# segasai/rvspecfit

Measured on AMD Instinct MI355X. Metric: spectra/sec (CCF+chi2 grid) DESI 3-arm, higher is better.
Workload: dtype f64

## Files before the change

rvspecfit_amd/csrc/ccf.hip:

```cpp
#include "common.h"

#define PP_NT 512
#define PP_LOG2NT 9
#define PP_NW (PP_NT / 64)


#define SEL_NB PP_NT
struct SelShared {
  unsigned long long kmin, kmax, result, next, cand[64];
  int hist[SEL_NB];
  int wtot[PP_NW];
  int cnt, nnan, nc, bucket, kk, nle;
};
__device__ __forceinline__ unsigned long long sel_key(double x) {
  const unsigned long long b = (unsigned long long)__double_as_longlong(x);
  return (b >> 63) ? ~b : (b | 0x8000000000000000ull);
}
__device__ __forceinline__ double sel_value(unsigned long long k) {
  const unsigned long long b = (k >> 63) ? (k & 0x7fffffffffffffffull) : ~k;
  return __longlong_as_double((long long)b);
}
__device__ __forceinline__ unsigned long long shfl_xor_u64(unsigned long long v,
                                                           int o) {
  const int lo = __shfl_xor((int)(v & 0xffffffffu), o, 64);
  const int hi = __shfl_xor((int)(v >> 32), o, 64);
  return ((unsigned long long)(unsigned)hi << 32) | (unsigned)lo;
}

__device__ double block_median(const double *v, int n, bool skipnan,
                               SelShared &Q) {
  const int tid = threadIdx.x, lane = tid & 63, wv = tid >> 6;
  {
    int cnt = 0, nn = 0;
    unsigned long long mn = ~0ull, mx = 0ull;
    for (int k = tid; k < n; k += PP_NT) {
      const double x = v[k];
      if (x != x) {
        nn++;
        continue;
      }
      const unsigned long long key = sel_key(x);
      cnt++;
      mn = key < mn ? key : mn;
      mx = key > mx ? key : mx;
    }
    cnt = wave_sum_i(cnt);
    nn = wave_sum_i(nn);
#pragma unroll
    for (int o = 32; o > 0; o >>= 1) {
      const unsigned long long a = shfl_xor_u64(mn, o), b = shfl_xor_u64(mx, o);
      mn = a < mn ? a : mn;
      mx = b > mx ? b : mx;
    }
    if (tid == 0) {
      Q.cnt = 0;
      Q.nnan = 0;
      Q.kmin = ~0ull;
      Q.kmax = 0ull;
    }
    __syncthreads();
    if (lane == 0) {
      atomicAdd(&Q.cnt, cnt);
      atomicAdd(&Q.nnan, nn);
      atomicMin(&Q.kmin, mn);
      atomicMax(&Q.kmax, mx);
    }
    __syncthreads();
  }
  const int nval = Q.cnt;
  if (nval == 0 || (!skipnan && Q.nnan > 0)) {
    __syncthreads();
    return __builtin_nan("");
  }
  const int k_lo = (nval - 1) >> 1, k_hi = nval >> 1;
  unsigned long long lo = Q.kmin, range = Q.kmax - Q.kmin;
  int kk = k_lo, ncand = nval;
  __syncthreads();
  unsigned long long found = 0;
  bool done = false;
  if (range == 0) {
    found = lo;
    done = true;
  }
  while (!done) {
    const int bits = 64 - __clzll((long long)range);
    const int shift = bits > PP_LOG2NT ? bits - PP_LOG2NT : 0;
    if (ncand <= 64) {
      if (tid == 0) Q.nc = 0;
      __syncthreads();
      for (int k = tid; k < n; k += PP_NT) {
        const double x = v[k];
        if (x != x) continue;
        const unsigned long long key = sel_key(x);
        if (key >= lo && key - lo <= range) Q.cand[atomicAdd(&Q.nc, 1)] = key;
      }
      __syncthreads();
      if (wv == 0) {
        const int nc = Q.nc;
        const unsigned long long my = lane < nc ? Q.cand[lane] : ~0ull;
        int lt = 0, eq = 0;
        for (int j = 0; j < nc; j++) {
          const unsigned long long c = Q.cand[j];
          lt += c < my;
          eq += c == my;
        }
        if (lane < nc && lt <= kk && kk < lt + eq) Q.result = my;
      }
      __syncthreads();
      found = Q.result;
      break;
    }
    Q.hist[tid] = 0;
    __syncthreads();
    for (int k = tid; k < n; k += PP_NT) {
      const double x = v[k];
      if (x != x) continue;
      const unsigned long long key = sel_key(x);
      if (key >= lo && key - lo <= range)
        atomicAdd(&Q.hist[(int)((key - lo) >> shift)], 1);
    }
    __syncthreads();
    const int h = Q.hist[tid];
    int inc = h;
#pragma unroll
    for (int o = 1; o < 64; o <<= 1) {
      const int t = __shfl_up(inc, o, 64);
      if (lane >= o) inc += t;
    }
    if (lane == 63) Q.wtot[wv] = inc;
    __syncthreads();
    int off = 0;
    for (int w = 0; w < wv; w++) off += Q.wtot[w];
    inc += off;
    if (inc - h <= kk && kk < inc) {
      Q.bucket = tid;
      Q.kk = kk - (inc - h);
      Q.nc = h;
    }
    __syncthreads();
    const int bsel = Q.bucket;
    kk = Q.kk;
    ncand = Q.nc;
    lo += (unsigned long long)bsel << shift;
    if (shift == 0) {
      found = lo;
      break;
    }
    range = (1ull << shift) - 1;
    __syncthreads();
  }
  double med = sel_value(found);
  if (k_hi != k_lo) {
    int nle = 0;
    unsigned long long nx = ~0ull;
    for (int k = tid; k < n; k += PP_NT) {
      const double x = v[k];
      if (x != x) continue;
      const unsigned long long key = sel_key(x);
      if (key <= found)
        nle++;
      else
        nx = key < nx ? key : nx;
    }
    nle = wave_sum_i(nle);
#pragma unroll
    for (int o = 32; o > 0; o >>= 1) {
      const unsigned long long a = shfl_xor_u64(nx, o);
      nx = a < nx ? a : nx;
    }
    __syncthreads();
    if (tid == 0) {
      Q.nle = 0;
      Q.next = ~0ull;
    }
    __syncthreads();
    if (lane == 0) {
      atomicAdd(&Q.nle, nle);
      atomicMin(&Q.next, nx);
    }
    __syncthreads();
    const double hi = (Q.nle >= k_hi + 1) ? med : sel_value(Q.next);
    med = (med + hi) * 0.5;
  }
  __syncthreads();
  return med;
}

__device__ __forceinline__ double wave_median256(const double (&x)[4], int cnt) {
  const int lane = threadIdx.x & 63;
  unsigned long long key[4];
  bool anynan = false;
#pragma unroll
  for (int h = 0; h < 4; h++) {
    const bool valid = lane + 64 * h < cnt;
    anynan |= valid && (x[h] != x[h]);
    key[h] = valid ? sel_key(x[h]) : ~0ull;
  }
  if (cnt <= 0 || __ballot(anynan) != 0ull) return __builtin_nan("");
  const int k_lo = (cnt - 1) >> 1, k_hi = cnt >> 1;
  unsigned long long p = 0;
  for (int bit = 63; bit >= 0; bit--) {
    const unsigned long long trial = p | (1ull << bit);
    int c = 0;
#pragma unroll
    for (int h = 0; h < 4; h++) c += __popcll(__ballot(key[h] < trial));
    if (c <= k_lo) p = trial;
  }
  double med = sel_value(p);
  if (k_hi != k_lo) {
    int cle = 0;
    unsigned long long nx = ~0ull;
#pragma unroll
    for (int h = 0; h < 4; h++) {
      const bool valid = lane + 64 * h < cnt;
      cle += __popcll(__ballot(valid && key[h] <= p));
      if (valid && key[h] > p && key[h] < nx) nx = key[h];
    }
#pragma unroll
    for (int o = 32; o > 0; o >>= 1) {
      const unsigned long long a = shfl_xor_u64(nx, o);
      nx = a < nx ? a : nx;
    }
    const double hi = (cle >= k_hi + 1) ? med : sel_value(nx);
    med = (med + hi) * 0.5;
  }
  return med;
}

__device__ __forceinline__ double median11_net(const double *w) {
  double a[11];
#pragma unroll
  for (int i = 0; i < 11; i++) a[i] = w[i];
#define CE(i, j)                         \
  {                                      \
    const double lo_ = fmin(a[i], a[j]); \
    a[j] = fmax(a[i], a[j]);             \
    a[i] = lo_;                          \
  }
  CE(0, 9) CE(1, 6) CE(2, 4) CE(3, 7) CE(5, 8)
  CE(0, 1) CE(3, 5) CE(4, 10) CE(6, 9) CE(7, 8)
  CE(1, 3) CE(2, 5) CE(4, 7) CE(8, 10)
  CE(0, 4) CE(1, 2) CE(3, 7) CE(5, 9) CE(6, 8)
  CE(2, 6) CE(4, 5) CE(7, 8)
  CE(2, 4) CE(3, 6) CE(5, 7)
  CE(3, 4) CE(5, 6)
  CE(4, 5)
#undef CE
  return a[5];
}

__device__ __forceinline__ double median11(double *a) {
#pragma unroll
  for (int i = 1; i < 11; i++) {
    const double x = a[i];
    int j = i - 1;
    while (j >= 0 && a[j] > x) {
      a[j + 1] = a[j];
      j--;
    }
    a[j + 1] = x;
  }
  return a[5];
}

#ifdef RVS_PP_TIMING
__device__ unsigned long long pp_dbg[16];
#define PP_T(i)                                                  \
  do {                                                           \
    __syncthreads();                                             \
    if (threadIdx.x == 0) {                                      \
      const unsigned long long t_ = wall_clock64();              \
      atomicAdd(&pp_dbg[i], t_ - t_prev);                        \
      t_prev = t_;                                               \
    }                                                            \
  } while (0)
extern "C" int rvs_dbg_read_pp(unsigned long long *out) {
  return hipMemcpyFromSymbol(out, HIP_SYMBOL(pp_dbg), sizeof(pp_dbg)) ==
                 hipSuccess
             ? 0
             : -1;
}
#define PP_TPARAM , unsigned long long &t_prev
#define PP_TPASS , t_prev
#else
#define PP_T(i)
#define PP_TPARAM
#define PP_TPASS
#endif

#define CCF_MAXNODE 24
#ifndef RVS_LM_MAXIT
#define RVS_LM_MAXIT 60
#endif

#define CCF_MODEL_MAXNODE 48
template <int MN>
struct LMSharedT {
  double p[MN];
  double c[MN], cn[MN], dl[MN];
  double bvec[MN];
  double Bd[MN * 3];
  double Lb[MN * 3];
  double isum[MN * 9];
  double red[PP_NW];
  double lamd, medv, mederr, medspec;
  int flag, ngood, firstgood, lastgood, nval, stop, ok;
};
typedef LMSharedT<CCF_MAXNODE> LMShared;
struct ErrArray {
  const double *ce;
  __device__ __forceinline__ double operator()(int k, double) const { return ce[k]; }
};


struct LMPix {
  double e0, e1, e2;
  int l;
};
#ifndef LM_PIX
#define LM_PIX 1
#endif

template <class LM, class ERR>
__device__ __forceinline__ double lm_eval(
    LM &S, const double *cc, const double *__restrict__ Eb,
    const int32_t *__restrict__ El, int npix, const double *cs, const ERR ce,
    double *wm, bool store, const LMPix (&px)[LM_PIX]) {
  __syncthreads();
  double c = 0;
#pragma unroll
  for (int i = 0; i < LM_PIX; i++) {
    const int k = threadIdx.x + i * PP_NT;
    if (k < npix) {
      const int l = px[i].l;
      double s = px[i].e0 * cc[l];
      s = fma(px[i].e1, cc[l + 1], s);
      s = fma(px[i].e2, cc[l + 2], s);
      const bool clipped = (s < -100.0) || (s > 100.0);
      s = fmin(fmax(s, -100.0), 100.0);
      const double mod = exp(s);
      const double sk = cs[k], e = ce(k, sk);
      const double f = (mod - sk) / e;
      const double z = f * f;
      const double r = sqrt(1 + z);
      c += 2 * (r - 1);
      if (store) wm[k] = clipped ? 0.0 : mod;
    }
  }
  for (int k = threadIdx.x + LM_PIX * PP_NT; k < npix; k += PP_NT) {
    const int l = El[k];
    double s = Eb[3 * k] * cc[l];
    s = fma(Eb[3 * k + 1], cc[l + 1], s);
    s = fma(Eb[3 * k + 2], cc[l + 2], s);
    const bool clipped = (s < -100.0) || (s > 100.0);
    s = fmin(fmax(s, -100.0), 100.0);
    const double mod = exp(s);
    const double sk = cs[k], e = ce(k, sk);
    const double f = (mod - sk) / e;
    const double z = f * f;
    const double r = sqrt(1 + z);
    c += 2 * (r - 1);
    if (store) wm[k] = clipped ? 0.0 : mod;
  }
  return 0.5 * block_sum<PP_NW>(c, S.red);
}

template <class LM, class ERR>
__device__ void lm_normal(LM &S, const double *__restrict__ Eb,
                          const int32_t *__restrict__ istart, int m,
                          const double *wm, const double *cs, const ERR ce) {
  const int nint = m - 2;
  const int lane = threadIdx.x & 63, wave = threadIdx.x >> 6;
  __syncthreads();
  for (int t = wave; t < nint; t += PP_NW) {
    double a[9];
#pragma unroll
    for (int q = 0; q < 9; q++) a[q] = 0;
    const int k1 = istart[t + 1];
    for (int k0 = istart[t] + lane; k0 < k1; k0 += 4 * 64) {
      double e[4][3];
#pragma unroll
      for (int c = 0; c < 4; c++) {
        const int k = min(k0 + 64 * c, k1 - 1);
        e[c][0] = Eb[3 * k];
        e[c][1] = Eb[3 * k + 1];
        e[c][2] = Eb[3 * k + 2];
      }
#pragma unroll
      for (int c = 0; c < 4; c++) {
        const int k = k0 + 64 * c;
        if (k < k1) {
          const double e0 = e[c][0], e1 = e[c][1], e2 = e[c][2];
          const double mod = wm[k], sk = cs[k], e = ce(k, sk);
          const double f = (mod - sk) / e;
          const double z = f * f;
          const double r = sqrt(1 + z);
          const double d = mod / e;
          const double h = d * d / (r * r * r), gg = d * f / r;
          a[0] = fma(h * e0, e0, a[0]);
          a[1] = fma(h * e0, e1, a[1]);
          a[2] = fma(h * e0, e2, a[2]);
          a[3] = fma(h * e1, e1, a[3]);
          a[4] = fma(h * e1, e2, a[4]);
          a[5] = fma(h * e2, e2, a[5]);
          a[6] = fma(gg, e0, a[6]);
          a[7] = fma(gg, e1, a[7]);
          a[8] = fma(gg, e2, a[8]);
        }
      }
    }
#pragma unroll
    for (int q = 0; q < 9; q++) {
      const double v = wave_sum_to63(a[q]);
      if (lane == 63) S.isum[t * 9 + q] = v;
    }
  }
  __syncthreads();
  for (int e = threadIdx.x; e < 4 * m; e += PP_NT) {
    const int a = e >> 2, d = e & 3;
    if (d == 3) {
      double s = 0;
      for (int t = max(0, a - 2); t <= min(a, nint - 1); t++)
        s += S.isum[t * 9 + 6 + (a - t)];
      S.bvec[a] = s;
    } else {
      const int lo = a - d;
      double s = 0;
      if (lo >= 0) {
        for (int t = max(0, a - 2); t <= min(lo, nint - 1); t++) {
          const int u = lo - t, v = a - t;
          const int idx = (u == 0) ? v : (u == 1 ? 2 + v : 5);
          s += S.isum[t * 9 + idx];
        }
      }
      S.Bd[a * 3 + d] = s;
    }
  }
  __syncthreads();
}

__device__ inline double lane_get(double v, int src) {
  return __hiloint2double(__builtin_amdgcn_readlane(__double2hiint(v), src),
                          __builtin_amdgcn_readlane(__double2loint(v), src));
}
__device__ inline double lane_put(double dst, double v, int lane) {
  return ((int)(threadIdx.x & 63) == lane) ? v : dst;
}

template <class LM>
__device__ void lm_band_solve(LM &S, int m) {
  const int lane = threadIdx.x & 63;
  const int r = min(lane, m - 1);
  const double ld = 1.0 + S.lamd;
  const double ra0 = S.Bd[r * 3] * ld, ra1 = S.Bd[r * 3 + 1],
               ra2 = S.Bd[r * 3 + 2], rb = S.bvec[r];
  double d1 = 0, d2 = 0, l1p = 0;
  double r1 = 0, r2 = 0;
  double z1 = 0, z2 = 0;
  double lb1 = 0, lb2 = 0, w = 0;
  bool ok = true;
  for (int i = 0; i < m; i++) {
    const double a0 = lane_get(ra0, i), a1 = lane_get(ra1, i),
                 a2 = lane_get(ra2, i), bi = lane_get(rb, i);
    const double l2 = (i >= 2) ? a2 * r2 : 0.0;
    const double l1 = (i >= 1) ? (a1 - l2 * l1p * d2) * r1 : 0.0;
    const double d = a0 - l1 * l1 * d1 - l2 * l2 * d2;
    if (!(d > 0)) ok = false;
    const double z = -bi - l1 * z1 - l2 * z2;
    const double rd = 1.0 / d;
    lb1 = lane_put(lb1, l1, i);
    lb2 = lane_put(lb2, l2, i);
    w = lane_put(w, z * rd, i);
    d2 = d1;
    d1 = d;
    r2 = r1;
    r1 = rd;
    l1p = l1;
    z2 = z1;
    z1 = z;
  }
  double x1 = 0, x2 = 0;
  double xs = 0;
  for (int i = m - 1; i >= 0; i--) {
    const double l1n = (i + 1 < m) ? lane_get(lb1, i + 1) : 0.0;
    const double l2n = (i + 2 < m) ? lane_get(lb2, i + 2) : 0.0;
    const double x = lane_get(w, i) - l1n * x1 - l2n * x2;
    xs = lane_put(xs, x, i);
    x2 = x1;
    x1 = x;
  }
  if (lane < m) {
    const double dl = ok ? xs : 0.0;
    S.dl[lane] = dl;
    S.cn[lane] = S.c[lane] + dl;
  }
  if (lane == 0) S.ok = ok ? 1 : 0;
}

template <class LM>
__device__ __forceinline__ void lm_binned_start(LM &S, SelShared &Q, const double *cs,
                                                const int32_t *__restrict__ bin_start,
                                                int m, bool f32) {
  const int tid = threadIdx.x;
  bool small = true;
  for (int jb = 0; jb < m; jb++)
    if (bin_start[jb + 1] - bin_start[jb] > 256) small = false;
  if (small) {
    const int lane = tid & 63, wv = tid >> 6;
    for (int jb = wv; jb < m; jb += PP_NW) {
      const int b0 = bin_start[jb], cnt = bin_start[jb + 1] - b0;
      double x[4];
#pragma unroll
      for (int h = 0; h < 4; h++) {
        const int q = lane + 64 * h;
        x[h] = (q < cnt) ? cs[b0 + q] : 0.0;
      }
      double stat = wave_median256(x, cnt);
      if (f32) stat = (double)(float)stat;
      if (lane == 0) {
        double p0 = log(fmax(stat, 1e-3 * S.medspec));
        if (!(stat == stat)) p0 = stat;
        if (!(fabs(p0) <= 1.79e308)) p0 = log(S.medspec);
        S.p[jb] = p0;
      }
    }
  } else {
    for (int jb = 0; jb < m; jb++) {
      const int b0 = bin_start[jb], cnt = bin_start[jb + 1] - b0;
      double stat = block_median(cs + b0, cnt, false, Q);
      if (f32) stat = (double)(float)stat;
      if (tid == 0) {
        double p0 = log(fmax(stat, 1e-3 * S.medspec));
        if (!(stat == stat)) p0 = stat;
        if (!(fabs(p0) <= 1.79e308)) p0 = log(S.medspec);
        S.p[jb] = p0;
      }
    }
  }
  __syncthreads();
}

template <class LM, class ERR>
__device__ __forceinline__ void lm_fit(LM &S, const double *__restrict__ Eb,
                                       const int32_t *__restrict__ El,
                                       const double *__restrict__ Cinv,
                                       const int32_t *__restrict__ istart, int m,
                                       int npix, const double *cs, const ERR ce,
                                       double *wm PP_TPARAM) {
  const int tid = threadIdx.x;
  if (tid < m) {
    double s = 0;
    for (int jj = 0; jj < m; jj++) s = fma(Cinv[tid * m + jj], S.p[jj], s);
    S.c[tid] = s;
  }
  if (tid == 0) {
#ifndef RVS_LM_LAMBDA0
#define RVS_LM_LAMBDA0 1e-3
#endif
    S.lamd = RVS_LM_LAMBDA0;
    S.stop = 0;
  }
  LMPix px[LM_PIX];
#pragma unroll
  for (int i = 0; i < LM_PIX; i++) {
    const int k = min(tid + i * PP_NT, npix - 1);
    px[i].e0 = Eb[3 * k];
    px[i].e1 = Eb[3 * k + 1];
    px[i].e2 = Eb[3 * k + 2];
    px[i].l = El[k];
  }
  double cost = lm_eval(S, S.c, Eb, El, npix, cs, ce, wm, true, px);
  PP_T(7);
  for (int it = 0; it < RVS_LM_MAXIT; it++) {
    lm_normal(S, Eb, istart, m, wm, cs, ce);
    PP_T(8);
    if (it == 0) {
      if (tid < 64) {
        double g = 0;
        if (tid < m)
          for (int i = 0; i < m; i++) g = fma(Cinv[i * m + tid], S.bvec[i], g);
        g = fabs(g);
        if (!(g == g)) g = 1.0;
        for (int o = 32; o > 0; o >>= 1) g = fmax(g, __shfl_xor(g, o));
        if (tid == 0 && g < 1e-8) S.stop = 1;
      }
      __syncthreads();
      if (S.stop) break;
    }
    bool accepted = false;
    for (int tries = 0; tries < 40; tries++) {
      if (tid < 64) lm_band_solve(S, m);
      PP_T(9);
      const double cn =
          lm_eval(S, S.cn, Eb, El, npix, cs, ce, wm, true, px);
      PP_T(10);
      if (cn <= cost) {
        accepted = true;
        double mx = 0;
        for (int i = 0; i < m; i++) mx = fmax(mx, fabs(S.dl[i]));
        const double rel = (cost - cn) / fmax(cost, 1e-300);
        __syncthreads();
        if (tid == 0) {
          for (int i = 0; i < m; i++) S.c[i] = S.cn[i];
          S.lamd = fmax(S.lamd / 8, 1e-12);
          if (mx < 1e-9 || rel < 1e-12) S.stop = 1;
        }
        cost = cn;
        break;
      }
      __syncthreads();
      if (tid == 0) {
        S.lamd *= 4;
        if (S.lamd > 1e12) S.stop = 1;
      }
      __syncthreads();
      if (S.stop) break;
    }
    __syncthreads();
    if (S.stop) break;
    if (!accepted)
      cost = lm_eval(S, S.c, Eb, El, npix, cs, ce, wm, true, px);
    PP_T(11);
  }
  __syncthreads();
}

__global__ void __launch_bounds__(PP_NT)
    __attribute__((amdgpu_waves_per_eu(4, 4)))
    ccf_preprocess_kernel(const double *__restrict__ lam,
                          const double *__restrict__ spec,
                          const double *__restrict__ espec,
                          const uint8_t *__restrict__ badmask, int npix,
                          int continuum, const double *__restrict__ Eb,
                          const int32_t *__restrict__ El,
                          const double *__restrict__ Cinv,
                          const int32_t *__restrict__ istart, int nnode,
                          const int32_t *__restrict__ bin_start,
                          const int32_t *__restrict__ xind,
                          const double *__restrict__ rw, int nfft, double maxerr,
                          double *__restrict__ proc_spec,
                          double *__restrict__ proc_ivar, double *__restrict__ sse,
                          double *__restrict__ cont_out,
                          double *__restrict__ pfit, int32_t *__restrict__ status,
                          const int32_t *__restrict__ gid,
                          const int32_t *__restrict__ npix_g,
                          const int32_t *__restrict__ nnode_g) {
  extern __shared__ double sm[];
  const int npix_s = npix, nnode_s = nnode;
  if (gid) {
    const int g = gid[blockIdx.x];
    npix = npix_g[g];
    nnode = nnode_g[g];
    lam += (int64_t)g * npix_s;
    xind += (int64_t)g * nfft;
    rw += (int64_t)g * nfft;
    if (continuum) {
      Eb += (int64_t)g * 3 * npix_s;
      El += (int64_t)g * npix_s;
      Cinv += (int64_t)g * 2 * nnode_s * nnode_s;
      istart += (int64_t)g * nnode_s;
      bin_start += (int64_t)g * (nnode_s + 1);
    }
  }
  double *cs = sm;
  double *ce = cs + npix;
  double *wm = ce + npix;
  uint8_t *msk = reinterpret_cast<uint8_t *>(wm + npix);
  __shared__ LMShared S;
  __shared__ SelShared Q;
  const int b = blockIdx.x, tid = threadIdx.x;
  const double *sp0 = spec + (int64_t)b * npix_s;
  const double *es0 = espec + (int64_t)b * npix_s;
#ifdef RVS_PP_TIMING
  unsigned long long t_prev = wall_clock64();
#endif

  for (int k = tid; k < npix; k += PP_NT) {
    cs[k] = sp0[k];
    ce[k] = es0[k];
    msk[k] = badmask ? (badmask[(int64_t)b * npix_s + k] != 0) : 0;
  }
  if (tid == 0) {
    S.flag = 0;
    S.nval = 0;
  }
  __syncthreads();

  {
    const double me = block_median(ce, npix, true, Q);
    if (tid == 0) S.mederr = me;
    __syncthreads();
  }
  const double mederr = S.mederr;

  if (continuum) {
    for (int k = tid; k < npix; k += PP_NT) {
      double w[11];
#pragma unroll
      for (int q = 0; q < 11; q++) {
        const int idx = k + q - 5;
        w[q] = (idx >= 0 && idx < npix) ? cs[idx] : 0.0;
      }
      bool hasnan = false;
#pragma unroll
      for (int q = 0; q < 11; q++) hasnan |= (w[q] != w[q]);
      const double med = hasnan ? median11(w) : median11_net(w);
      if ((ce[k] > maxerr * mederr) || (med <= 0)) msk[k] = 1;
    }
  }
  __syncthreads();
  PP_T(0);
  {
    int ng = 0, fg = npix, lg = -1;
    for (int k = tid; k < npix; k += PP_NT) {
      if (msk[k]) {
        ce[k] = 1e9 * mederr;
      } else {
        ng++;
        fg = min(fg, k);
        lg = max(lg, k);
      }
    }
    ng = wave_sum_i(ng);
#pragma unroll
    for (int o = 32; o > 0; o >>= 1) {
      fg = min(fg, __shfl_xor(fg, o, 64));
      lg = max(lg, __shfl_xor(lg, o, 64));
    }
    if (tid == 0) {
      S.ngood = 0;
      S.firstgood = npix;
      S.lastgood = -1;
    }
    __syncthreads();
    if ((tid & 63) == 0) {
      atomicAdd(&S.ngood, ng);
      atomicMin(&S.firstgood, fg);
      atomicMax(&S.lastgood, lg);
    }
    __syncthreads();
    if (S.ngood == 0) {
      if (tid == 0) S.flag |= RVS_ST_ALLMASKED;
      for (int k = tid; k < npix; k += PP_NT)
        if (!(fabs(cs[k]) <= 1.79e308)) cs[k] = 1;
    } else {
      const int fgood = S.firstgood, lgood = S.lastgood;
      for (int k = tid; k < npix; k += PP_NT) {
        if (!msk[k]) continue;
        double val;
        if (k < fgood)
          val = sp0[fgood];
        else if (k > lgood)
          val = sp0[lgood];
        else {
          int a = k - 1, c = k + 1;
          while (msk[a]) a--;
          while (msk[c]) c++;
          const double l1 = lam[a], l2 = lam[c], l0 = lam[k];
          val = (-(l1 - l0) * sp0[c] + (l2 - l0) * sp0[a]) / (l2 - l1);
        }
        cs[k] = val;
      }
    }
    __syncthreads();
  }

  PP_T(1);
  {
    const double md = block_median(cs, npix, false, Q);
    if (tid == 0) {
      S.medv = md;
      double ms = md;
      if (ms <= 0) {
        ms = fabs(ms);
        if (ms == 0) ms = 1;
      }
      S.medspec = ms;
    }
    __syncthreads();
  }
  const double medv = S.medv;

  if (continuum) {
    const int m = nnode;
    PP_T(2);
    lm_binned_start(S, Q, cs, bin_start, m, false);

    PP_T(3);
    lm_fit(S, Eb, El, Cinv, istart, m, npix, cs, ErrArray{ce}, wm PP_TPASS);
    if (pfit && tid < m) {
      const double *Cm = Cinv + m * m;
      double s = 0;
      for (int jj = 0; jj < m; jj++) s = fma(Cm[tid * m + jj], S.c[jj], s);
      pfit[(int64_t)b * nnode_s + tid] = s;
    }
  }

  PP_T(4);
  for (int k = tid; k < npix; k += PP_NT) {
    double cont = 1.0;
    if (continuum) {
      const int l = El[k];
      double s = Eb[3 * k] * S.c[l];
      s = fma(Eb[3 * k + 1], S.c[l + 1], s);
      s = fma(Eb[3 * k + 2], S.c[l + 2], s);
      cont = exp(fmin(fmax(s, -100.0), 100.0));
    }
    if (medv > 0)
      cont = fmax(1e-2 * medv, cont);
    else
      cont = fmax(cont, 1.0);
    if (cont_out) cont_out[(int64_t)b * npix_s + k] = cont;
    const double e = ce[k];
    double iv = 1.0 / (e * e);
    double c = sp0[k] / cont;
    iv = cont * cont * iv;
    if (msk[k]) {
      iv = 0;
      c = 0;
    }
    cs[k] = c;
    ce[k] = iv;
  }
  __syncthreads();
  PP_T(5);
  double ss = 0;
  for (int n = tid; n < nfft; n += PP_NT) {
    const int xi = xind[n];
    double r1 = 0, r2 = 0;
    if (xi >= 0) {
      const double rwt = rw[n], lwt = 1 - rwt;
      r1 = lwt * cs[xi] + rwt * cs[xi + 1];
      const double a = ce[xi], c = ce[xi + 1];
      r2 = a * c / (lwt * lwt * c + rwt * rwt * a + ((a * c) == 0 ? 1.0 : 0.0));
    }
    proc_spec[(int64_t)b * nfft + n] = r1;
    proc_ivar[(int64_t)b * nfft + n] = r2;
    ss += r1 * r1 * r2;
  }
  ss = block_sum<PP_NW>(ss, S.red);
  if (tid == 0) {
    sse[b] = ss;
    if (S.flag && status) atomicOr(&status[b], S.flag);
  }
  PP_T(6);
}

extern "C" int rvs_ccf_preprocess_g(const double *lam, const double *spec,
                                  const double *espec, const uint8_t *badmask,
                                  int npix, int B, int continuum,
                                  const double *Eb, const int32_t *El,
                                  const double *Cinv, const int32_t *istart,
                                  int nnode, const int32_t *bin_start,
                                  const int32_t *xind, const double *rw, int nfft,
                                  double maxerr, double *proc_spec,
                                  double *proc_ivar, double *sse, double *cont,
                                  double *pfit, int32_t *status,
                                  const int32_t *grid_id,
                                  const int32_t *npix_g, const int32_t *nnode_g,
                                  void *stream) {
  if (npix < 12 || B < 1 || nfft < 2) return RVS_E_ARG;
  if (grid_id && (!npix_g || (continuum && !nnode_g))) return RVS_E_ARG;
  if (continuum && (nnode < 3 || nnode > CCF_MAXNODE)) return RVS_E_ARG;
  const size_t shm = sizeof(double) * 3 * (size_t)npix + ((npix + 15) / 16) * 16;
  if (shm + sizeof(LMShared) + sizeof(SelShared) > 159 * 1024) return RVS_E_ARG;
  static bool attr_set = false;
  if (!attr_set) {
    (void)hipFuncSetAttribute((const void *)ccf_preprocess_kernel,
                              hipFuncAttributeMaxDynamicSharedMemorySize,
                              (int)(159 * 1024 - sizeof(LMShared) - sizeof(SelShared)));
    (void)hipGetLastError();
    attr_set = true;
  }
  hipLaunchKernelGGL(ccf_preprocess_kernel, dim3(B), dim3(PP_NT), shm,
                     rvs_stream(stream), lam, spec, espec, badmask, npix,
                     continuum, Eb, El, Cinv, istart, nnode, bin_start, xind, rw,
                     nfft, maxerr, proc_spec, proc_ivar, sse, cont, pfit, status, grid_id,
                     npix_g, nnode_g);
  RVS_LAUNCH_CHECK();
  return 0;
}

extern "C" int rvs_ccf_preprocess(const double *lam, const double *spec,
                                  const double *espec, const uint8_t *badmask,
                                  int npix, int B, int continuum,
                                  const double *Eb, const int32_t *El,
                                  const double *Cinv, const int32_t *istart,
                                  int nnode, const int32_t *bin_start,
                                  const int32_t *xind, const double *rw, int nfft,
                                  double maxerr, double *proc_spec,
                                  double *proc_ivar, double *sse, double *cont,
                                  double *pfit, int32_t *status, void *stream) {
  return rvs_ccf_preprocess_g(lam, spec, espec, badmask, npix, B, continuum, Eb, El,
                              Cinv, istart, nnode, bin_start, xind, rw, nfft, maxerr,
                              proc_spec, proc_ivar, sse, cont, pfit, status, nullptr,
                              nullptr, nullptr, stream);
}

struct ErrModel {
  const double *es;
  double floor_;
  bool f32;
  __device__ __forceinline__ double operator()(int k, double s) const {
    if (es) return es[k];
    if (f32) return (double)fmaxf(__fmul_rn((float)s, 1e-5f), (float)floor_);
    return fmax(s * 1e-5, floor_);
  }
};
typedef LMSharedT<CCF_MODEL_MAXNODE> LMSharedModel;
#define CCF_MODEL_LDS (159 * 1024)
static_assert(sizeof(double) * 2 * RVS_CCF_MODEL_MAX_NTP + sizeof(LMSharedModel) +
                      sizeof(SelShared) <= CCF_MODEL_LDS,
              "a model row of RVS_CCF_MODEL_MAX_NTP pixels does not fit the LDS");

__global__ void __launch_bounds__(PP_NT)
    ccf_model_kernel(const double *__restrict__ rows,
                     const uint8_t *__restrict__ f32row,
                     const double *__restrict__ erows, int ntp, int continuum,
                     const double *__restrict__ Eb, const int32_t *__restrict__ El,
                     const double *__restrict__ Cinv,
                     const int32_t *__restrict__ istart, int nnode,
                     const int32_t *__restrict__ bin_start,
                     const double *__restrict__ lnlam,
                     const double *__restrict__ logl,
                     const int32_t *__restrict__ ihi, int npoints,
                     double *__restrict__ model, double *__restrict__ cont_out,
                     double *__restrict__ pfit, int32_t *__restrict__ status) {
  extern __shared__ double sm[];
  double *cs = sm;
  double *wm = cs + ntp;
  __shared__ LMSharedModel S;
  __shared__ SelShared Q;
  const int b = blockIdx.x, tid = threadIdx.x;
  const double *row = rows + (int64_t)b * ntp;
  const bool f32 = f32row && f32row[b] != 0;
  for (int k = tid; k < ntp; k += PP_NT) cs[k] = row[k];
  __syncthreads();
  const double *y = cs;
  if (continuum) {
    const int m = nnode;
    {
      double md = block_median(cs, ntp, false, Q);
      if (f32) md = (double)(float)md;
      if (tid == 0) {
        S.medv = md;
        double ms = md;
        if (ms <= 0) {
          ms = fabs(ms);
          if (ms == 0) ms = 1;
          if (status) atomicOr(&status[b], RVS_ST_NONPOS_MEDIAN);
        }
        S.medspec = ms;
      }
      __syncthreads();
    }
    const ErrModel ce = {erows ? erows + (int64_t)b * ntp : nullptr, 1e-2 * S.medv,
                         f32};
    lm_binned_start(S, Q, cs, bin_start, m, f32);
#ifdef RVS_PP_TIMING
    unsigned long long t_prev = wall_clock64();
#endif
    lm_fit(S, Eb, El, Cinv, istart, m, ntp, cs, ce, wm PP_TPASS);
    if (pfit && tid < m) {
      const double *Cm = Cinv + m * m;
      double s = 0;
      for (int jj = 0; jj < m; jj++) s = fma(Cm[tid * m + jj], S.c[jj], s);
      pfit[(int64_t)b * nnode + tid] = s;
    }
    for (int k = tid; k < ntp; k += PP_NT) {
      const int l = El[k];
      double s = Eb[3 * k] * S.c[l];
      s = fma(Eb[3 * k + 1], S.c[l + 1], s);
      s = fma(Eb[3 * k + 2], S.c[l + 2], s);
      const double cont = exp(fmin(fmax(s, -100.0), 100.0));
      wm[k] = cont;
      if (cont_out) cont_out[(int64_t)b * ntp + k] = cont;
    }
    __syncthreads();
    const double cfloor = 1e-2 * block_median(wm, ntp, false, Q);
    for (int k = tid; k < ntp; k += PP_NT) {
      double cont = wm[k];
      cont = (cfloor != cfloor) ? cfloor : fmax(cont, cfloor);
      wm[k] = cs[k] / cont;
    }
    __syncthreads();
    y = wm;
  }
  const bool d32 = f32 && !continuum;
  for (int n = tid; n < npoints; n += PP_NT) {
    const int hi = ihi[n];
    double v = 1.0;
    if (hi >= 1 && hi < ntp) {
      const double ylo = y[hi - 1], yhi = y[hi], xlo = lnlam[hi - 1];
      const double dy = d32 ? (double)__fsub_rn((float)yhi, (float)ylo) : yhi - ylo;
      const double slope = dy / (lnlam[hi] - xlo);
      v = slope * (logl[n] - xlo) + ylo;
    }
    model[(int64_t)b * npoints + n] = v;
  }
}

__global__ void __launch_bounds__(256)
    ccf_model_rows_kernel(const float *__restrict__ dats, int64_t ngrid,
                          const int64_t *__restrict__ sel, int exp_flag, int ntp,
                          double *__restrict__ rows) {
  const int b = blockIdx.x;
  const int64_t r = sel[b];
  const bool ok = r >= 0 && r < ngrid;
  const float *src = dats + (ok ? r : 0) * ntp;
  for (int k = threadIdx.x; k < ntp; k += 256) {
    double v = __builtin_nan("");
    if (ok) v = exp_flag ? (double)np_expf(src[k]) : (double)src[k];
    rows[(int64_t)b * ntp + k] = v;
  }
}

extern "C" int rvs_ccf_model_rows(const float *dats, int64_t ngrid, const int64_t *sel,
                                  int exp_flag, int ntp, int M, double *rows,
                                  void *stream) {
  if (!dats || !sel || !rows || ngrid < 1 || ntp < 1 || M < 1) return RVS_E_ARG;
  hipLaunchKernelGGL(ccf_model_rows_kernel, dim3(M), dim3(256), 0, rvs_stream(stream),
                     dats, ngrid, sel, exp_flag, ntp, rows);
  RVS_LAUNCH_CHECK();
  return 0;
}

int ccf_model_rfft(const double *model, int nfft, int M, const double *twid,
                   double *fft, double *fft2, hipStream_t st);

extern "C" int rvs_ccf_models_build(const double *rows, const uint8_t *f32row,
                                    const double *erows, int ntp, int M,
                                    int continuum, const double *Eb,
                                    const int32_t *El, const double *Cinv,
                                    const int32_t *istart, int nnode,
                                    const int32_t *bin_start, const double *lnlam,
                                    const double *logl, const int32_t *ihi,
                                    int npoints, const double *twid, double *model,
                                    double *fft, double *fft2, double *cont,
                                    double *pfit, int32_t *status, void *stream) {
  if (ntp < 12 || ntp > RVS_CCF_MODEL_MAX_NTP || M < 1 || npoints < 2)
    return RVS_E_ARG;
  if (!rows || !lnlam || !logl || !ihi || !model) return RVS_E_ARG;
  if (continuum && (nnode < 3 || nnode > CCF_MODEL_MAXNODE || !Eb || !El || !Cinv ||
                    !istart || !bin_start))
    return RVS_E_ARG;
  if ((fft != nullptr) != (fft2 != nullptr)) return RVS_E_ARG;
  if (fft) {
    if (npoints < 64 || npoints > 16384 || (npoints & (npoints - 1)) || !twid)
      return RVS_E_ARG;
  }
  const size_t shm = sizeof(double) * 2 * (size_t)ntp;
  static bool attr_set = false;
  if (!attr_set) {
    (void)hipFuncSetAttribute(
        (const void *)ccf_model_kernel, hipFuncAttributeMaxDynamicSharedMemorySize,
        (int)(CCF_MODEL_LDS - sizeof(LMSharedModel) - sizeof(SelShared)));
    (void)hipGetLastError();
    attr_set = true;
  }
  hipLaunchKernelGGL(ccf_model_kernel, dim3(M), dim3(PP_NT), shm, rvs_stream(stream),
                     rows, f32row, erows, ntp, continuum, Eb, El, Cinv, istart, nnode,
                     bin_start, lnlam, logl, ihi, npoints, model, cont, pfit, status);
  RVS_LAUNCH_CHECK();
  if (fft) return ccf_model_rfft(model, npoints, M, twid, fft, fft2, rvs_stream(stream));
  return 0;
}

__global__ void __launch_bounds__(256)
    ccf_select_kernel(const double *__restrict__ chisq,
                      const double *__restrict__ sse, int narm, int T,
                      const double *__restrict__ vgrid, int nvel,
                      double *__restrict__ res, double *__restrict__ best_ccf,
                      int32_t *__restrict__ status) {
  __shared__ double sv[4];
  __shared__ long long sk[4];
  const int b = blockIdx.x, tid = threadIdx.x;
  double tot = 0;
  for (int a = 0; a < narm; a++) tot += sse[(int64_t)a * gridDim.x + b];
  const double *c = chisq + (int64_t)b * T * nvel;
  double bv = __builtin_inf();
  long long bk = (1ll << 62);
  for (int e = tid; e < T * nvel; e += 256) {
    const double x = c[e] + tot;
    if (nan_less(x, e, bv, bk)) {
      bv = x;
      bk = e;
    }
  }
#pragma unroll
  for (int o = 32; o > 0; o >>= 1) {
    const double ov = __shfl_xor(bv, o, 64);
    const long long ok = __shfl_xor(bk, o, 64);
    if (nan_less(ov, ok, bv, bk)) {
      bv = ov;
      bk = ok;
    }
  }
  if ((tid & 63) == 0) {
    sv[tid >> 6] = bv;
    sk[tid >> 6] = bk;
  }
  __syncthreads();
  bv = sv[0];
  bk = sk[0];
  for (int w = 1; w < 4; w++)
    if (nan_less(sv[w], sk[w], bv, bk)) {
      bv = sv[w];
      bk = sk[w];
    }
  const int best_id = (int)(bk / nvel);
  const double *row = c + (int64_t)best_id * nvel;
  for (int v = tid; v < nvel; v += 256)
    best_ccf[(int64_t)b * nvel + v] = row[v] + tot;
  if (tid == 0) {
    int bp = 0;
    double mv = row[0] + tot;
    for (int v = 1; v < nvel; v++) {
      const double x = row[v] + tot;
      if (nan_less(x, v, mv, bp)) {
        mv = x;
        bp = v;
      }
    }
    double vel = vgrid[bp];
    if (bp != 0 && bp != nvel - 1) {
      const double xa = vgrid[bp - 1], xb = vgrid[bp], xc = vgrid[bp + 1];
      const double ya = row[bp - 1] + tot, yb = row[bp] + tot, yc = row[bp + 1] + tot;
      const double d1 = (yb - ya) / (xb - xa), d2 = (yc - yb) / (xc - xb);
      const double a2 = (d2 - d1) / (xc - xa);
      if (a2 > 0) vel = xb - (d1 + a2 * (xb - xa)) / (2 * a2);
    }
    int st = 0;
    if (!(fabs(mv) <= 1.79e308)) st |= RVS_ST_CCF_FAILED;
    double *r = res + (int64_t)b * 4;
    r[0] = best_id;
    r[1] = vel;
    r[2] = bp;
    r[3] = mv;
    if (st && status) atomicOr(&status[b], st);
  }
}

extern "C" int rvs_ccf_select(const double *chisq, const double *sse,
                              int narm_sse, int B, int T, const double *vgrid,
                              int nvel, double *res, double *best_ccf,
                              int32_t *status, void *stream) {
  if (B < 1 || T < 1 || nvel < 1) return RVS_E_ARG;
  hipLaunchKernelGGL(ccf_select_kernel, dim3(B), dim3(256), 0,
                     rvs_stream(stream), chisq, sse, narm_sse, T, vgrid, nvel,
                     res, best_ccf, status);
  RVS_LAUNCH_CHECK();
  return 0;
}
```

Measured before the change: 83310.

## Fuse LM cost evaluation with normal-equation accumulation in one pixel pass

Merges the separate cost-evaluation pass and the normal-matrix build into one lm_pass that recomputes the model exp, the cost and the Hessian/gradient partial sums together, walking pixels by interval. The normal equations are now built for every trial point instead of only after an accepted step, and the wm shared-memory model buffer is dropped from the preprocess kernel. This saves a full pixel sweep and block barriers per LM iteration, and replaces sqrt and divides with rsqrt and a reciprocal, at the cost of doing normal-equation work on rejected trials. Shared memory per block shrinks, which may raise occupancy.

```diff
diff --git a/rvspecfit_amd/csrc/ccf.hip b/rvspecfit_amd/csrc/ccf.hip
--- a/rvspecfit_amd/csrc/ccf.hip
+++ b/rvspecfit_amd/csrc/ccf.hip
@@ -313,66 +313,17 @@
 };
 
 
-struct LMPix {
-  double e0, e1, e2;
-  int l;
-};
-#ifndef LM_PIX
-#define LM_PIX 1
-#endif
-
 template <class LM, class ERR>
-__device__ __forceinline__ double lm_eval(
-    LM &S, const double *cc, const double *__restrict__ Eb,
-    const int32_t *__restrict__ El, int npix, const double *cs, const ERR ce,
-    double *wm, bool store, const LMPix (&px)[LM_PIX]) {
-  __syncthreads();
-  double c = 0;
-#pragma unroll
-  for (int i = 0; i < LM_PIX; i++) {
-    const int k = threadIdx.x + i * PP_NT;
-    if (k < npix) {
-      const int l = px[i].l;
-      double s = px[i].e0 * cc[l];
-      s = fma(px[i].e1, cc[l + 1], s);
-      s = fma(px[i].e2, cc[l + 2], s);
-      const bool clipped = (s < -100.0) || (s > 100.0);
-      s = fmin(fmax(s, -100.0), 100.0);
-      const double mod = exp(s);
-      const double sk = cs[k], e = ce(k, sk);
-      const double f = (mod - sk) / e;
-      const double z = f * f;
-      const double r = sqrt(1 + z);
-      c += 2 * (r - 1);
-      if (store) wm[k] = clipped ? 0.0 : mod;
-    }
-  }
-  for (int k = threadIdx.x + LM_PIX * PP_NT; k < npix; k += PP_NT) {
-    const int l = El[k];
-    double s = Eb[3 * k] * cc[l];
-    s = fma(Eb[3 * k + 1], cc[l + 1], s);
-    s = fma(Eb[3 * k + 2], cc[l + 2], s);
-    const bool clipped = (s < -100.0) || (s > 100.0);
-    s = fmin(fmax(s, -100.0), 100.0);
-    const double mod = exp(s);
-    const double sk = cs[k], e = ce(k, sk);
-    const double f = (mod - sk) / e;
-    const double z = f * f;
-    const double r = sqrt(1 + z);
-    c += 2 * (r - 1);
-    if (store) wm[k] = clipped ? 0.0 : mod;
-  }
-  return 0.5 * block_sum<PP_NW>(c, S.red);
-}
-
-template <class LM, class ERR>
-__device__ void lm_normal(LM &S, const double *__restrict__ Eb,
-                          const int32_t *__restrict__ istart, int m,
-                          const double *wm, const double *cs, const ERR ce) {
+__device__ __forceinline__ double lm_pass(LM &S, const double *cc,
+                                          const double *__restrict__ Eb,
+                                          const int32_t *__restrict__ istart, int m,
+                                          const double *cs, const ERR ce) {
   const int nint = m - 2;
   const int lane = threadIdx.x & 63, wave = threadIdx.x >> 6;
   __syncthreads();
+  double cost = 0;
   for (int t = wave; t < nint; t += PP_NW) {
+    const double c0 = cc[t], c1 = cc[t + 1], c2 = cc[t + 2];
     double a[9];
 #pragma unroll
     for (int q = 0; q < 9; q++) a[q] = 0;
@@ -391,12 +342,21 @@
         const int k = k0 + 64 * c;
         if (k < k1) {
           const double e0 = e[c][0], e1 = e[c][1], e2 = e[c][2];
-          const double mod = wm[k], sk = cs[k], e = ce(k, sk);
-          const double f = (mod - sk) / e;
+          double s = e0 * c0;
+          s = fma(e1, c1, s);
+          s = fma(e2, c2, s);
+          const bool clipped = (s < -100.0) || (s > 100.0);
+          s = fmin(fmax(s, -100.0), 100.0);
+          const double mod = exp(s);
+          const double sk = cs[k], er = ce(k, sk);
+          const double ie = 1.0 / er;
+          const double f = (mod - sk) * ie;
           const double z = f * f;
-          const double r = sqrt(1 + z);
-          const double d = mod / e;
-          const double h = d * d / (r * r * r), gg = d * f / r;
+          const double rr = rsqrt(1 + z);
+          const double r = (1 + z) * rr;
+          cost += 2 * (r - 1);
+          const double dr = clipped ? 0.0 : mod * ie * rr;
+          const double h = dr * dr * rr, gg = dr * f;
           a[0] = fma(h * e0, e0, a[0]);
           a[1] = fma(h * e0, e1, a[1]);
           a[2] = fma(h * e0, e2, a[2]);
@@ -415,7 +375,12 @@
       if (lane == 63) S.isum[t * 9 + q] = v;
     }
   }
-  __syncthreads();
+  return 0.5 * block_sum<PP_NW>(cost, S.red);
+}
+
+template <class LM>
+__device__ __forceinline__ void lm_assemble(LM &S, int m) {
+  const int nint = m - 2;
   for (int e = threadIdx.x; e < 4 * m; e += PP_NT) {
     const int a = e >> 2, d = e & 3;
     if (d == 3) {
@@ -436,7 +401,6 @@
       S.Bd[a * 3 + d] = s;
     }
   }
-  __syncthreads();
 }
 
 __device__ inline double lane_get(double v, int src) {
@@ -542,11 +506,9 @@
 
 template <class LM, class ERR>
 __device__ __forceinline__ void lm_fit(LM &S, const double *__restrict__ Eb,
-                                       const int32_t *__restrict__ El,
                                        const double *__restrict__ Cinv,
                                        const int32_t *__restrict__ istart, int m,
-                                       int npix, const double *cs, const ERR ce,
-                                       double *wm PP_TPARAM) {
+                                       const double *cs, const ERR ce PP_TPARAM) {
   const int tid = threadIdx.x;
   if (tid < m) {
     double s = 0;
@@ -560,20 +522,11 @@
     S.lamd = RVS_LM_LAMBDA0;
     S.stop = 0;
   }
-  LMPix px[LM_PIX];
-#pragma unroll
-  for (int i = 0; i < LM_PIX; i++) {
-    const int k = min(tid + i * PP_NT, npix - 1);
-    px[i].e0 = Eb[3 * k];
-    px[i].e1 = Eb[3 * k + 1];
-    px[i].e2 = Eb[3 * k + 2];
-    px[i].l = El[k];
-  }
-  double cost = lm_eval(S, S.c, Eb, El, npix, cs, ce, wm, true, px);
+  double cost = lm_pass(S, S.c, Eb, istart, m, cs, ce);
+  lm_assemble(S, m);
+  __syncthreads();
   PP_T(7);
   for (int it = 0; it < RVS_LM_MAXIT; it++) {
-    lm_normal(S, Eb, istart, m, wm, cs, ce);
-    PP_T(8);
     if (it == 0) {
       if (tid < 64) {
         double g = 0;
@@ -590,10 +543,9 @@
     bool accepted = false;
     for (int tries = 0; tries < 40; tries++) {
       if (tid < 64) lm_band_solve(S, m);
+      PP_T(8);
+      const double cn = lm_pass(S, S.cn, Eb, istart, m, cs, ce);
       PP_T(9);
-      const double cn =
-          lm_eval(S, S.cn, Eb, El, npix, cs, ce, wm, true, px);
-      PP_T(10);
       if (cn <= cost) {
         accepted = true;
         double mx = 0;
@@ -605,6 +557,7 @@
           S.lamd = fmax(S.lamd / 8, 1e-12);
           if (mx < 1e-9 || rel < 1e-12) S.stop = 1;
         }
+        lm_assemble(S, m);
         cost = cn;
         break;
       }
@@ -618,9 +571,12 @@
     }
     __syncthreads();
     if (S.stop) break;
-    if (!accepted)
-      cost = lm_eval(S, S.c, Eb, El, npix, cs, ce, wm, true, px);
-    PP_T(11);
+    if (!accepted) {
+      cost = lm_pass(S, S.c, Eb, istart, m, cs, ce);
+      lm_assemble(S, m);
+      __syncthreads();
+    }
+    PP_T(10);
   }
   __syncthreads();
 }
@@ -664,8 +620,7 @@
   }
   double *cs = sm;
   double *ce = cs + npix;
-  double *wm = ce + npix;
-  uint8_t *msk = reinterpret_cast<uint8_t *>(wm + npix);
+  uint8_t *msk = reinterpret_cast<uint8_t *>(ce + npix);
   __shared__ LMShared S;
   __shared__ SelShared Q;
   const int b = blockIdx.x, tid = threadIdx.x;
@@ -787,7 +742,7 @@
     lm_binned_start(S, Q, cs, bin_start, m, false);
 
     PP_T(3);
-    lm_fit(S, Eb, El, Cinv, istart, m, npix, cs, ErrArray{ce}, wm PP_TPASS);
+    lm_fit(S, Eb, Cinv, istart, m, cs, ErrArray{ce} PP_TPASS);
     if (pfit && tid < m) {
       const double *Cm = Cinv + m * m;
       double s = 0;
@@ -862,8 +817,9 @@
   if (npix < 12 || B < 1 || nfft < 2) return RVS_E_ARG;
   if (grid_id && (!npix_g || (continuum && !nnode_g))) return RVS_E_ARG;
   if (continuum && (nnode < 3 || nnode > CCF_MAXNODE)) return RVS_E_ARG;
-  const size_t shm = sizeof(double) * 3 * (size_t)npix + ((npix + 15) / 16) * 16;
-  if (shm + sizeof(LMShared) + sizeof(SelShared) > 159 * 1024) return RVS_E_ARG;
+  const size_t admit = sizeof(double) * 3 * (size_t)npix + ((npix + 15) / 16) * 16;
+  if (admit + sizeof(LMShared) + sizeof(SelShared) > 159 * 1024) return RVS_E_ARG;
+  const size_t shm = sizeof(double) * 2 * (size_t)npix + ((npix + 15) / 16) * 16;
   static bool attr_set = false;
   if (!attr_set) {
     (void)hipFuncSetAttribute((const void *)ccf_preprocess_kernel,
@@ -928,7 +884,7 @@
                      double *__restrict__ pfit, int32_t *__restrict__ status) {
   extern __shared__ double sm[];
   double *cs = sm;
-  double *wm = cs + ntp;
+  double *yc = cs + ntp;
   __shared__ LMSharedModel S;
   __shared__ SelShared Q;
   const int b = blockIdx.x, tid = threadIdx.x;
@@ -960,7 +916,7 @@
 #ifdef RVS_PP_TIMING
     unsigned long long t_prev = wall_clock64();
 #endif
-    lm_fit(S, Eb, El, Cinv, istart, m, ntp, cs, ce, wm PP_TPASS);
+    lm_fit(S, Eb, Cinv, istart, m, cs, ce PP_TPASS);
     if (pfit && tid < m) {
       const double *Cm = Cinv + m * m;
       double s = 0;
@@ -973,18 +929,18 @@
       s = fma(Eb[3 * k + 1], S.c[l + 1], s);
       s = fma(Eb[3 * k + 2], S.c[l + 2], s);
       const double cont = exp(fmin(fmax(s, -100.0), 100.0));
-      wm[k] = cont;
+      yc[k] = cont;
       if (cont_out) cont_out[(int64_t)b * ntp + k] = cont;
     }
     __syncthreads();
-    const double cfloor = 1e-2 * block_median(wm, ntp, false, Q);
+    const double cfloor = 1e-2 * block_median(yc, ntp, false, Q);
     for (int k = tid; k < ntp; k += PP_NT) {
-      double cont = wm[k];
+      double cont = yc[k];
       cont = (cfloor != cfloor) ? cfloor : fmax(cont, cfloor);
-      wm[k] = cs[k] / cont;
-    }
-    __syncthreads();
-    y = wm;
+      yc[k] = cs[k] / cont;
+    }
+    __syncthreads();
+    y = yc;
   }
   const bool d32 = f32 && !continuum;
   for (int n = tid; n < npoints; n += PP_NT) {
```

After: 83230, median of 4. No clear change (-0.1%).
